# stivalaa/cuda_satabsearch

Measured on AMD Instinct MI355X. Metric: db-structure scorings/sec (query×db pairs/sec) at r=128; 1/2/4/8 MI355X, higher is better.
Workload: dtype i32

## Files before the change

### cuda_satabsearch_amd/build.py

```python
import os
import re
import shutil
import subprocess
import sys

PKG = os.path.dirname(os.path.abspath(__file__))
ROOT = os.path.dirname(PKG)
CSRC = os.path.join(PKG, "csrc")
HOST = os.path.join(CSRC, "host")
INC = os.path.join(ROOT, "include")

HIPCC = os.environ.get("HIPCC") or shutil.which("hipcc") or "/opt/rocm/bin/hipcc"
CC = os.environ.get("CC") or "gcc"


def _run(cmd):
    print("+", " ".join(cmd), flush=True)
    subprocess.run(cmd, check=True)


def _stale(target, sources):
    if not os.path.exists(target):
        return True
    t = os.path.getmtime(target)
    return any(os.path.getmtime(s) > t for s in sources)


DEVICE_SOURCES = ("sat_launch.hip", "sat_capi.hip", "sat_pairs.hip", "sat_db.hip", "sat_topk.hip", "sat_multi.hip",
                  "sat_polish.hip", "sat_qfromdb.hip", "sat_cluster.hip", "sat_eval.hip", "sat_cover.hip", "sat_profile.hip",
                  "sat_reorder.hip", "sat_exact.hip", "sat_reach.hip")
KERNEL_SOURCES = ("sat_sa_kernel.hpp", "sat_sa_body.inc", "sat_launch.hpp", "sat_launch.hip")
HIPFLAGS = ["--offload-arch=gfx950", "-O3", "-ffp-contract=off", "-std=c++17", "-fPIC", "-I", INC, "-I", CSRC]
DEVICE_LIB = (os.path.join(PKG, "libsatabsearch.so"), os.path.join(PKG, "obj", "lib"), [])
SELFCHECK_LIB = (os.path.join(ROOT, "tests", "native", "libsat_selfcheck.so"), os.path.join(PKG, "obj", "selfcheck"),
                 ["-DSAT_DIAG", "-DSAT_DIAG_SELFCHECK"])
JOBS = 16


def kernel_source_hash():
    import hashlib
    h = hashlib.sha256()
    for f in KERNEL_SOURCES:
        with open(os.path.join(CSRC, f), "rb") as fh:
            h.update(fh.read())
    return h.hexdigest()


def include_closure(src):
    seen, todo = [], [src]
    while todo:
        f = todo.pop()
        if f in seen:
            continue
        seen.append(f)
        with open(f) as fh:
            names = re.findall(r'^[ \t]*#[ \t]*include[ \t]+"([^"]+)"', fh.read(), re.M)
        for name in names:
            hits = [p for p in (os.path.normpath(os.path.join(d, name)) for d in (os.path.dirname(f), CSRC, INC)) if os.path.exists(p)]
            todo += hits[:1]
    return seen


def build_host(force=False):
    out = os.path.join(PKG, "libsathost.so")
    srcs = [os.path.join(HOST, f) for f in ("sat_parse.c", "sat_gumbel.c", "sat_shard.c", "sat_cluster.c", "sat_eval.c", "sat_cover.c",
                                            "sat_profile.c", "sat_reorder.c", "sat_exact.c", "sat_reach.c")]
    deps = srcs + [os.path.join(HOST, f) for f in ("sat_parse.h", "sat_gumbel.h", "sat_stats.h", "sat_shard.h", "sat_cluster.h", "sat_eval.h",
                                                "sat_cover.h", "sat_profile.h", "sat_reorder.h", "sat_exact.h", "sat_reach.h")]
    if force or _stale(out, deps):
        _run([CC, "-O2", "-fPIC", "-shared", "-Wall", "-Wextra", "-I", HOST, "-o", out] + srcs + ["-lm", "-lpthread"])
    return out


def _host_objects(force=False):
    host_c = [os.path.join(HOST, "sat_gumbel.c"), os.path.join(HOST, "sat_shard.c"), os.path.join(HOST, "sat_cluster.c"),
              os.path.join(HOST, "sat_eval.c"), os.path.join(HOST, "sat_cover.c"), os.path.join(HOST, "sat_reach.c")]
    host_o = [os.path.join(PKG, "sat_gumbel.o"), os.path.join(PKG, "sat_shard.o"), os.path.join(PKG, "sat_cluster.o"),
              os.path.join(PKG, "sat_eval.o"), os.path.join(PKG, "sat_cover.o"), os.path.join(PKG, "sat_reach.o")]
    for c, o in zip(host_c, host_o):
        if force or _stale(o, [c] + [os.path.join(HOST, h) for h in ("sat_gumbel.h", "sat_stats.h", "sat_shard.h", "sat_cluster.h", "sat_eval.h",
                                                                      "sat_cover.h", "sat_reach.h")]):
            _run([CC, "-O2", "-fPIC", "-ffp-contract=off", "-Wall", "-Wextra", "-I", HOST, "-c", "-o", o, c])
    return host_o


def build_device_libs(libs, force=False):
    host_c = [os.path.join(HOST, f) for f in ("sat_gumbel.c", "sat_shard.c", "sat_cluster.c", "sat_eval.c", "sat_cover.c",
                                              "sat_reach.c", "sat_gumbel.h", "sat_stats.h", "sat_shard.h", "sat_cluster.h",
                                              "sat_eval.h", "sat_cover.h", "sat_reach.h")]
    srcs = [os.path.join(CSRC, f) for f in DEVICE_SOURCES]
    deps = [include_closure(src) for src in srcs]
    todo = [lib for lib in libs if force or _stale(lib[0], host_c + sum(deps, []))]
    if not todo:
        return
    host_o = _host_objects(force)
    compiles = []
    for out, objdir, flags in todo:
        os.makedirs(objdir, exist_ok=True)
    for src, dep in zip(srcs, deps):
        for out, objdir, flags in todo:
            obj = os.path.join(objdir, os.path.splitext(os.path.basename(src))[0] + ".o")
            if force or _stale(obj, dep):
                compiles.append([HIPCC] + HIPFLAGS + flags + ["-c", "-o", obj, src])
    from concurrent.futures import ThreadPoolExecutor
    with ThreadPoolExecutor(JOBS) as ex:
        list(ex.map(_run, compiles))
    for out, objdir, flags in todo:
        objs = [os.path.join(objdir, os.path.splitext(f)[0] + ".o") for f in DEVICE_SOURCES]
        _run([HIPCC, "--offload-arch=gfx950", "-fPIC", "-shared", "-o", out] + ["-Wl," + o for o in objs + host_o] + ["-lm", "-ldl"])


def build_device(force=False):
    build_device_libs([DEVICE_LIB], force)
    return DEVICE_LIB[0]


def build_cli(force=False):
    src = os.path.join(HOST, "sat_main.c")
    if not os.path.exists(src):
        return None
    bindir = os.path.join(PKG, "bin")
    os.makedirs(bindir, exist_ok=True)
    out = os.path.join(bindir, "satabsearch")
    host_search = os.path.join(HOST, "sat_host_search.c")
    deps = [src, host_search, os.path.join(HOST, "sat_host_search.h"), os.path.join(HOST, "sat_cluster.h"),
            os.path.join(HOST, "sat_cover.h"), os.path.join(HOST, "sat_profile.h"), os.path.join(HOST, "sat_reorder.h"),
            os.path.join(PKG, "libsatabsearch.so"), os.path.join(PKG, "libsathost.so")]
    if force or _stale(out, deps):
        _run([CC, "-O3", "-ffp-contract=off", "-Wall", "-Wextra", "-I", INC, "-I", HOST, "-o", out, src, host_search,
              "-L", PKG, "-lsatabsearch", "-lsathost", "-lm", "-Wl,-rpath,$ORIGIN/.."])
    return out


def build_test_native(force=False, twin=True):
    tdir = os.path.join(ROOT, "tests", "native")
    src = os.path.join(tdir, "rocrand_check.hip")
    if not os.path.exists(src):
        return None
    out = os.path.join(tdir, "librocrand_check.so")
    if force or _stale(out, [src, os.path.join(CSRC, "sat_sa_kernel.hpp"), os.path.join(CSRC, "sat_sa_body.inc")]):
        _run([HIPCC, "--offload-arch=gfx950", "-O3", "-std=c++17", "-fPIC", "-shared", "-I", INC, "-I", CSRC, "-o", out, src])
    if twin:
        build_device_libs([SELFCHECK_LIB], force)
    src2, out2 = os.path.join(tdir, "lds_residency.hip"), os.path.join(tdir, "liblds_residency.so")
    if os.path.exists(src2) and (force or _stale(out2, [src2])):
        _run([HIPCC, "--offload-arch=gfx950", "-O2", "-std=c++17", "-fPIC", "-shared", "-o", out2, src2])
    src3, out3 = os.path.join(tdir, "stream_probe.hip"), os.path.join(tdir, "libstream_probe.so")
    if os.path.exists(src3) and (force or _stale(out3, [src3])):
        _run([HIPCC, "--offload-arch=gfx950", "-O2", "-std=c++17", "-fPIC", "-shared", "-o", out3, src3])
    return out


def build_oracle(ref=False):
    odir = os.path.join(ROOT, "oracle")
    _run(["make", "-s", "-C", odir, "all"])
    if ref and os.path.isdir("/root/reference/nvcc_src_current"):
        _run(["make", "-s", "-C", odir, "ref"])


def build_all(force=False, oracle=False, ref=False):
    build_host(force)
    if oracle:
        build_device_libs([DEVICE_LIB, SELFCHECK_LIB], force)
        build_test_native(force, twin=False)
        build_cli(force)
        build_oracle(ref)
    else:
        build_device(force)
        build_cli(force)


if __name__ == "__main__":
    build_all(force="--force" in sys.argv, oracle="--oracle" in sys.argv or "--ref" in sys.argv,
              ref="--ref" in sys.argv)
```

### cuda_satabsearch_amd/csrc/sat_sa_body.inc

```
    using namespace satk;
    constexpr int M1W = (N1P + 31) / 32;
    extern __shared__ __align__(16) unsigned char lds_raw[];

    const int nthreads = a.tpe;
    const int wave_wg = __builtin_amdgcn_readfirstlane((int)(threadIdx.x >> 6));
    const int slot = a.epw > 1 ? wave_wg / (nthreads >> 6) : 0;
    const int wlane = (int)(threadIdx.x & 63u);
    const int lane_id = ((wave_wg - slot * (nthreads >> 6)) << 6) | wlane;
    __builtin_assume(lane_id >= 0 && lane_id < 1024);
    const uint32_t lds_base = (uint32_t)slot * a.lds_stride;
    unsigned char *const lds_slot = lds_raw + lds_base;
    constexpr bool FAST = OPT >= 0;
    const int lpc_shift = FAST ? (OPT >> 2) : a.lpc_shift;
    const bool opt_lorder = FAST ? (OPT & 1) != 0 : a.lorder != 0;
    const bool opt_compact = FAST ? (OPT & 1) != 0 : a.compact != 0;
    const int lpc = 1 << lpc_shift;
    const int tid = lane_id >> lpc_shift;
    const int part = lane_id & (lpc - 1);
    const int T = nthreads >> lpc_shift;
    const int list_pos = (int)blockIdx.x * a.epw + slot;
    SatPairItem pit{};
    if constexpr (PAIRS) pit = px.items[min(list_pos, a.n_list - 1)];
    const int e = PAIRS ? pit.entry : a.entry_list[min(list_pos, a.n_list - 1)];
    const SatQuery Q = PAIRS ? a.queries[pit.desc] : a.queries[blockIdx.y];
// ... 165 lines not shown
        }
        __syncthreads();
    }

    uint8_t *smap_b = reinterpret_cast<uint8_t *>(smap);
    uint8_t *bmap_b = reinterpret_cast<uint8_t *>(bmap);
    auto bmap_byte_addr = [&](int k) -> int { return (__mul24(k >> 2, T) + tid) * 4 + (k & 3); };
    const int T4 = TP << 2, tid4 = tid << 2;
    auto map_byte_addr = [&](int k) -> int { return __mul24(k >> 2, T4) + tid4 + (k & 3); };

    auto score_rows = [&]() -> int {
        int total = 0;
        for (int i = 0; i < n1 - 1; i++) {
            const uint32_t jb = smap_b[map_byte_addr(i)];
            const int j = MAPOFF ? (int)(jb >> 3) : (int)jb;
            const bool jreal = MAPOFF ? (jb & SAT_MAP_UNMATCHED) == 0u : j != NULLJ;
            const DbRow<CELLS> drow = db_row(jreal ? j : 0);
            int rowsum = 0;
            auto row_group = [&](int kw) {
                const int below = i + 1 - 4 * kw;
                const uint32_t force = below <= 0 ? 0u : (0x04040404u >> (8 * (4 - below)));
                const uint32_t qi = (uint32_t)(kw * N1P + i);
                rowsum = quad_terms(load_qdist(qi << 4), load_qcode(qi << 2), drow, smap[kw * TP + tid], force, rowsum);
            };
            if (lpc == 1) {
                for (int kw = (i + 1) >> 2; kw < n1w; kw++) {
                    const int below = i + 1 - 4 * kw;
                    const uint32_t force = below <= 0 ? 0u : (0x04040404u >> (8 * (4 - below)));
                    const uint32_t qi = (uint32_t)(kw * N1P + i);
                    rowsum = quad_terms(load_qdist_uniform(qi), load_qcode_uniform(qi), drow, smap[kw * TP + tid], force, rowsum);
                }
            } else {
                for (int kw = ((i + 1) >> 2) + part; kw < n1w; kw += lpc) row_group(kw);
            }
            total += jreal ? rowsum : 0;
        }
        return total;
    };

    const uint64_t subseq_lo = (uint64_t)a.ordinal[e];
    int best = SAT_K_NO_SCORE;
    uint32_t best_restart = 0xFFFFFFFFu;
    bool any = false;

    const int cmp_recip = (65536 + cmp_lpi - 1) / cmp_lpi;
    const int per_round = (64 * cmp_recip) >> 16;
    const int sub = __mul24(wlane, cmp_recip) >> 16, kw = wlane - __mul24(sub, cmp_lpi);
    const bool lane_ok = sub < per_round;
    const int tail1_recip = (65536 + n1w - 1) / n1w, tail1_rows = (64 * tail1_recip) >> 16;
    const int tail2_lpi = (n1w + 1) >> 1;
    const int tail2_recip = (65536 + tail2_lpi - 1) / tail2_lpi;
    const int tail2_rows = 2 * tail2_lpi <= cmp_words ? (64 * tail2_recip) >> 16 : 0;
    const uint32_t nullword = map_encode<MAPOFF>(NULLJ, NULLJ) * 0x01010101u;
    SAT_PHASE(7);
    SAT_DIAG_PERTURB_INIT;
    size_t mrow = 0;
    uint32_t *mrec = nullptr;
    int r_begin = tid, r_end = a.maxstart;
    if constexpr (PAIRS) {
        r_begin = pit.r0 + tid;
        r_end = pit.r1;
    }
    int rbest = SAT_K_NO_SCORE;
    Bits<M2W> rset = bits_zero<M2W>();
    if constexpr (MATCH) {
        if constexpr (PAIRS) {
            mrow = (size_t)pit.pair;
            mrec = mx.rec_slabs + (size_t)pit.slab * mx.rec_slab_words;
        } else {
            mrow = (size_t)(&a.queries[blockIdx.y] - mx.desc_base) * (size_t)mx.n_entries + (size_t)e;
            mrec = mx.rec_slabs + ((size_t)blockIdx.y * gridDim.x * a.epw + list_pos) * mx.rec_slab_words;
        }
        if (replay) {
            const int cnt = mx.counts[mrow];
            r_begin = tid < cnt ? mx.restarts[mrow * mx.max_matches + tid] : 0;
            r_end = tid < cnt ? r_begin + 1 : 0;
        }
    }
    for (int restart = r_begin; restart < r_end; restart += T) {
        any = true;
        SAT_PHASE(7);
        const uint64_t subseq = subseq_lo | ((uint64_t)(uint32_t)restart << 32);

        Bits<M1W> mapped = bits_zero<M1W>();
        Bits<M2W> occ = bits_zero<M2W>();
        {
            {
                int wa = tid;
                asm volatile("" : "+v"(wa));
                for (int w = 0; w < cmp_words; w++, wa += TP) smap[wa] = nullword;
            }
            int j = 0;
            bool stopped = false;
            for (int i0 = 0; i0 < n1; i0 += 4) {
                if constexpr (N1P > 32)
                    if (__builtin_amdgcn_ballot_w64(!stopped) == 0ull) break;
                uint4 r = philox_block(Q.seed_q, subseq, (uint32_t)(i0 >> 2));
                uint32_t rv[4] = { r.x, r.y, r.z, r.w };
#pragma unroll
                for (int s = 0; s < 4; s++) {
                    const int i = i0 + s;
                    if (i < n1) {
                        if (!stopped && rv[s] < 0x7FFFFFC0u) {
                            Bits<M2W> cand, below = bits_below<M2W>(j);
                            if constexpr (M2W == 1) {
                                cand.w[0] = qmask[i] & ~below.w[0];
                            } else {
                                const int t = qtypes[i];
#pragma unroll
                                for (int w = 0; w < M2W; w++) cand.w[w] = tmask[t * TMS + w] & ~below.w[w];
                            }
                            int jj = bits_lowest<M2W>(cand);
                            if (jj < 0) {
                                stopped = true;
                            } else {
                                smap_b[map_byte_addr(i)] = (uint8_t)(MAPOFF ? jj << 3 : jj);
                                bits_set<M1W>(mapped, i);
                                bits_set<M2W>(occ, jj);
                                j = jj + 1;
                            }
                        }
                    }
                }
            }
        }

        SAT_PHASE(10);
        int score = 0;
        constexpr bool FS_PAIRS = N1P > 16 && !SAT_DIAG_FS_ROWS_ONLY;
        bool walk_pairs = FS_PAIRS;
        if constexpr (FS_PAIRS) {
            constexpr int PAIR_COST = 27;
            const int m = bits_count<M1W>(mapped);
            walk_pairs = __builtin_amdgcn_ballot_w64(__mul24(__mul24(m, m - 1), PAIR_COST) > __mul24(__mul24(n1w, n1), 31)) == 0ull;
        }
        if (walk_pairs) {
            typedef uint32_t u32x2_t __attribute__((ext_vector_type(2)));
            typedef const __attribute__((address_space(1))) u32x2_t *gptr_u2;
            const gptr_c qpairG = (gptr_c)(uintptr_t)Q.qpair;
            constexpr bool POP_IMAGES = M2W == 1;
            static_assert(POP_IMAGES || !MAPOFF, "the walk's map-byte reads take plain indices");
            Bits<M1W> ri = mapped;
            Bits<M2W> rj = occ;
            auto pop = [](auto &b, bool &valid) -> int {
                constexpr int W = sizeof(b.w) / sizeof(b.w[0]);
                valid = bits_any<W>(b);
                const int pos = max(bits_lowest<W>(b), 0);
                bits_drop_lowest<W>(b);
                return pos;
            };
            constexpr bool FS_TEAMS = SAT_FS_TEAMS && M1W == 1 && M2W == 1 && FAST && (OPT == 0 || OPT == 1);
            bool teamed = false;
            if constexpr (FS_TEAMS) teamed = __builtin_amdgcn_ballot_w64(true) == ~0ull;
            if (FS_TEAMS && teamed) {
                const int pl = wlane & 1;
                const uint32_t om = (uint32_t)__shfl_xor((int)mapped.w[0], 1, 64), oo = (uint32_t)__shfl_xor((int)occ.w[0], 1, 64);
                const uint32_t m0 = pl ? om : mapped.w[0], o0 = pl ? oo : occ.w[0];
                const uint32_t m1 = pl ? mapped.w[0] : om, o1 = pl ? occ.w[0] : oo;
                const int c0n = __popc(m0), c1n = __popc(m1);
                const bool big1 = c1n > c0n;
                const uint32_t mb = big1 ? m1 : m0, ob = big1 ? o1 : o0, msm = big1 ? m0 : m1, osm = big1 ? o0 : o1;
                const int rb = max((big1 ? c1n : c0n) - 1, 0), rs = max((big1 ? c0n : c1n) - 1, 0);
                const int dlead = rb - rs, etot = rb + rs;
                uint32_t rm = mb, ro = ob;
                int cur = 0, acc_b = 0, acc_s = 0;
                bool on_small = false;
                for (int e = pl; __builtin_amdgcn_ballot_w64(e < etot) != 0ull; e += 2) {
                    const bool act = e < etot;
                    const int e2 = e - dlead;
                    const bool small = e2 >= 0 && (e2 & 1) != 0;
                    const int len = e2 < 0 ? rb - e : rs - (e2 >> 1);
                    const int a = (small ? rs : rb) - len;
                    if (small && !on_small) { rm = msm; ro = osm; cur = 0; on_small = true; }
#pragma unroll
                    for (int q = 0; q < 2; q++) {
                        const uint32_t go = (act && cur < a) ? 1u : 0u;
                        rm &= rm - go;
                        ro &= ro - go;
                        cur += (int)go;
                    }
                    const int i = act ? __ffs(rm) - 1 : 0, ji = act ? __ffs(ro) - 1 : 0;
                    Bits<1> rk, rl;
                    rk.w[0] = act ? rm & (rm - 1u) : 0u;
                    rl.w[0] = act ? ro & (ro - 1u) : 0u;
                    const DbRow<CELLS> drow = db_row(ji);
                    const uint32_t qrow = (uint32_t)__mul24(i, N1P * 8);
                    int rowsum = 0;
                    while (__builtin_amdgcn_ballot_w64(rk.w[0] != 0u) != 0ull) {
                        int ll[SAT_FS_UNROLL];
                        bool vv[SAT_FS_UNROLL];
                        u32x2_t qcell[SAT_FS_UNROLL];
#pragma unroll
                        for (int u = 0; u < SAT_FS_UNROLL; u++) {
                            bool vl;
                            const int k = pop(rk, vv[u]);
                            ll[u] = pop(rl, vl);
                            qcell[u] = *(gptr_u2)(qpairG + (qrow + ((uint32_t)k << 3)));
                        }
#pragma unroll
                        for (int u = 0; u < SAT_FS_UNROLL; u++) {
                            const uint2 c = db_cell<CELLS>(drow, ll[u]);
                            const int term = pair_term(qcell[u].x, qcell[u].y, c.x, c.y);
                            rowsum += vv[u] ? term : 0;
                        }
                    }
                    acc_s += small ? rowsum : 0;
                    acc_b += small ? 0 : rowsum;
                }
                const int acc0 = big1 ? acc_s : acc_b, acc1 = big1 ? acc_b : acc_s;
                score = (pl ? acc1 : acc0) + __shfl_xor(pl ? acc0 : acc1, 1, 64);
            } else
            while (__builtin_amdgcn_ballot_w64(bits_any<M1W>(ri)) != 0ull) {
                bool ai, aj;
                int i = 0, ji = 0;
                ai = false;
                Bits<M1W> rk = bits_zero<M1W>();
                Bits<M2W> rl = bits_zero<M2W>();
                for (int p = 0; p < lpc; p++) {
                    bool v;
                    const int pos = pop(ri, v);
                    int img = 0;
                    if constexpr (POP_IMAGES) { bool vj; img = pop(rj, vj); }
                    if (p == part) {
                        i = pos;
                        ai = v;
                        ji = img;
                        rk = ri;
                        rl = rj;
                    }
                }
                (void)aj;
                if constexpr (!POP_IMAGES) { ji = smap_b[map_byte_addr(i)]; ji = ai ? ji : 0; }
                const DbRow<CELLS> drow = db_row(ji);
                const uint32_t qrow = (uint32_t)__mul24(i, N1P * 8);
                int rowsum = 0;
                while (__builtin_amdgcn_ballot_w64(bits_any<M1W>(rk)) != 0ull) {
                    int ll[SAT_FS_UNROLL];
                    bool vv[SAT_FS_UNROLL];
                    u32x2_t qcell[SAT_FS_UNROLL];
#pragma unroll
                    for (int u = 0; u < SAT_FS_UNROLL; u++) {
                        const int ku = pop(rk, vv[u]);
                        ll[u] = 0;
                        if constexpr (POP_IMAGES) { bool vl; ll[u] = pop(rl, vl); }
                        if constexpr (!POP_IMAGES) ll[u] = smap_b[map_byte_addr(ku)];
                        qcell[u] = *(gptr_u2)(qpairG + (qrow + ((uint32_t)ku << 3)));
                    }
#pragma unroll
                    for (int u = 0; u < SAT_FS_UNROLL; u++) {
                        const uint2 c = db_cell<CELLS>(drow, ll[u]);
                        const int term = pair_term(qcell[u].x, qcell[u].y, c.x, c.y);
                        rowsum += vv[u] ? term : 0;
                    }
                }
                score += rowsum;
            }
        } else {
            score = score_rows();
        }
        if (lpc >= 2) score += __shfl_xor(score, 1, 64);
        if (lpc == 4) score += __shfl_xor(score, 2, 64);
        const int best_before = best;
        if (score > best) {
            best = score;
            if (lsoln && beats_leader(score, restart))
                for (int w = 0; w < n1w; w++) bmap[w * T + tid] = smap[w * TP + tid];
        }
        if constexpr (MATCH) {
            rbest = score;
            rset = occ;
            if (replay && part == 0)
                for (int w = 0; w < n1w; w++) bmap[w * T + tid] = smap[w * TP + tid];
        }

        SAT_PHASE(6);
        uint4 blk = uint4{ 0u, 0u, 0u, 0u };
        for (int iter = 0; iter < SAT_K_MAXITER; iter++) {
            const int rowoff = prowC[2 * iter], rowmax = prowC[2 * iter + 1];
            constexpr bool ROW_IN_LANES = N1P >= 32 && M2W == 1 && (OPT < 0 || (OPT & 1) != 0);
            float rowv = 0.0f;
            if constexpr (ROW_IN_LANES)
                rowv = *(gptr_f32)((gptr_c)ptabG + (((uint32_t)rowoff + (uint32_t)min(wlane, rowmax + 2)) << 2));
            if ((iter & 1) == 0) {
                blk = philox_block(Q.seed_q, subseq, (uint32_t)(SAT_K_STEP_BLOCK0 + (iter >> 1)));
            } else {
                blk.x = blk.z;
                blk.y = blk.w;
            }
            const uint32_t word_a = blk.x, word_b = blk.y;
            SAT_DIAG_PERTURB_STEP;

            const int ssei = scaled_index16(word_a >> 16, n1, n1 - 1);

            int oldj;
            Bits<M2W> cand;
            int rank_base = 0;
            if (M2W == 1 && opt_lorder) {
                int p;
                bool none;
                highest_mapped_upto(mapped, ssei, p, none);
                const int A = MAPOFF ? smap_b[map_byte_addr(p)] >> 3 : smap_b[map_byte_addr(p)];
                SAT_DIAG_DUP_MAPBYTE(&smap_b[map_byte_addr(p)]);
                oldj = (p == ssei && !(MAPOFF && none)) ? A : NULLJ;
                const uint32_t above = 0xFFFFFFFEu << (A & 31);
                const uint32_t y = occ.w[0] & above;
                const uint32_t gap = (y - 1u) & ~y & above;
                const bool empty = none || (y == 0u && ssei != n1 - 1);
// ... 390 lines not shown
```

### cuda_satabsearch_amd/csrc/sat_sa_kernel.hpp

```cpp
#pragma once

#include <hip/hip_runtime.h>
#include <type_traits>
#include <stdint.h>

#ifdef SAT_DIAG
#include "diag/sat_diag.hpp"
#endif
#ifndef SAT_DIAG_ARGS
#define SAT_DIAG_ARGS
#endif
#ifndef SAT_PHASE_INIT
#define SAT_PHASE_INIT
#define SAT_PHASE(k)
#define SAT_PHASE_FLUSH
#endif
#ifndef SAT_DIAG_FS_ROWS_ONLY
#define SAT_DIAG_FS_ROWS_ONLY 0
#endif
#ifndef SAT_DIAG_DUP_CELLS
#define SAT_DIAG_DUP_CELLS(row, o0, o1, o2, o3)
#endif
#ifndef SAT_DIAG_DUP_MAPWORD
#define SAT_DIAG_DUP_MAPWORD(p)
#endif
#ifndef SAT_DIAG_DUP_ATOMIC
#define SAT_DIAG_DUP_ATOMIC(p)
#endif
#ifndef SAT_DIAG_DUP_MAPBYTE
#define SAT_DIAG_DUP_MAPBYTE(p)
#endif
#ifndef SAT_DIAG_PERTURB_INIT
#define SAT_DIAG_PERTURB_INIT
#define SAT_DIAG_PERTURB_STEP
#define SAT_DIAG_PERTURB_END
#endif
#ifndef SAT_DIAG_SELFCHECK_STEP
#define SAT_DIAG_SELFCHECK_STEP
#endif

#define SAT_CELLS_FULL8 0
#define SAT_CELLS_FULL5 1
#define SAT_CELLS_TRI5  2
#ifndef SAT_FAST_WAVES
#define SAT_FAST_WAVES 6
#endif
#ifndef SAT_FS_TEAMS
#define SAT_FS_TEAMS 1
#endif
#ifndef SAT_PICK_TABLE
#define SAT_PICK_TABLE 1
#endif
#define SAT_K_MAXITER 100
#define SAT_K_MAXDIM 111
#define SAT_FS_UNROLL 2
#define SAT_K_STEP_BLOCK0 32
#define SAT_K_EPS 1.1e-7
#define SAT_K_NO_SCORE (-99999)
#define SAT_K_QSENT 1.0e30f
#define SAT_K_DSENT (-1.0e30f)

struct SatQuery {
    const float4   *qdist;
    const uint32_t *qcode;
    const uint8_t  *qtypes;
    const uint2    *qpair;
    int32_t         n1;
    uint32_t        pad_;
    uint64_t        seed_q;
    int32_t        *scores;
    int8_t         *ssemaps;
};

struct SatKernelArgs {
    const int32_t  *orders;
    const int64_t  *cell_off;
    const uint8_t  *tab_tri;
    const float    *dist_tri;
    const uint32_t *ordinal;
    const int32_t  *entry_list;
    int32_t         n_list;
    int32_t         epw, tpe;
    uint32_t        lds_stride;
    const SatQuery *queries;
    int32_t         lorder, lsoln, maxstart;
    int32_t         lpc_shift;
    int32_t         compact;
    uint32_t       *bmap_slabs;
    uint32_t        bmap_slab_words;
    const float    *ptab;
    const int32_t  *prow;
    SAT_DIAG_ARGS
};

struct SatMatchArgs {
    const SatQuery *desc_base;
    int32_t         n_entries;
    int32_t         max_matches;
    int32_t         replay;
    int32_t         map_pitch;
    uint32_t       *rec_slabs;
    uint32_t        rec_slab_words;
    uint32_t        pad_;
    int32_t        *counts;
    int32_t        *scores;
    int32_t        *restarts;
    int8_t         *maps;
};

struct SatPairItem {
    int32_t pair;
    int32_t desc;
    int32_t entry;
    int32_t r0, r1;
    int32_t slab;
    int32_t pad_[2];
};
struct SatPairArgs {
    const SatPairItem   *items;
    unsigned long long  *keys;
    int8_t              *maps;
};

namespace satk {

template <int W> struct Bits { uint32_t w[W]; };

template <int W> __device__ __forceinline__ Bits<W> bits_zero()
{
    Bits<W> b;
#pragma unroll
    for (int i = 0; i < W; i++) b.w[i] = 0u;
    return b;
}
template <int W> __device__ __forceinline__ Bits<W> bits_below(int pos)
{
    Bits<W> b;
    if constexpr (W == 1) {
        const int s = 32 - min(max(pos, 0), 32);
        const int h = s >> 1;
        b.w[0] = (0xFFFFFFFFu >> h) >> (s - h);
        return b;
    }
    const int wi = pos >> 5;
    const uint32_t part = (1u << (pos & 31)) - 1u;
#pragma unroll
    for (int i = 0; i < W; i++) b.w[i] = i < wi ? 0xFFFFFFFFu : (i == wi ? part : 0u);
    return b;
}
template <int W> __device__ __forceinline__ void bits_set(Bits<W> &b, int pos)
{
#pragma unroll
    for (int i = 0; i < W; i++) b.w[i] |= ((pos >> 5) == i) ? (1u << (pos & 31)) : 0u;
}
template <int W> __device__ __forceinline__ void bits_clear(Bits<W> &b, int pos)
{
#pragma unroll
    for (int i = 0; i < W; i++) b.w[i] &= ~(((pos >> 5) == i) ? (1u << (pos & 31)) : 0u);
}
template <int W> __device__ __forceinline__ int bits_count(const Bits<W> &b)
{
    int c = 0;
#pragma unroll
    for (int i = 0; i < W; i++) c += __popc(b.w[i]);
    return c;
}
template <int W> __device__ __forceinline__ bool bits_any(const Bits<W> &b)
{
    uint32_t o = 0u;
#pragma unroll
    for (int i = 0; i < W; i++) o |= b.w[i];
    return o != 0u;
}
template <int W> __device__ __forceinline__ void bits_drop_lowest(Bits<W> &b)
{
    bool done = false;
#pragma unroll
    for (int i = 0; i < W; i++) {
        const bool here = !done && b.w[i] != 0u;
        b.w[i] = here ? b.w[i] & (b.w[i] - 1u) : b.w[i];
        done = done || here;
    }
}
template <int W> __device__ __forceinline__ int bits_lowest(const Bits<W> &b)
{
    int r = -1;
#pragma unroll
    for (int i = W - 1; i >= 0; i--) r = b.w[i] ? 32 * i + (__ffs(b.w[i]) - 1) : r;
    return r;
}
template <int W> __device__ __forceinline__ int bits_highest(const Bits<W> &b)
{
    int r = -1;
#pragma unroll
    for (int i = 0; i < W; i++) r = b.w[i] ? 32 * i + (31 - __clz(b.w[i])) : r;
    return r;
}
__device__ __forceinline__ int word_select(uint32_t v, int r)
{
    uint32_t a = v - ((v >> 1) & 0x55555555u);
    uint32_t b = (a & 0x33333333u) + ((a >> 2) & 0x33333333u);
// ... 149 lines not shown
        const uint64_t p0 = (uint64_t)0xD2511F53u * c0, p1 = (uint64_t)0xCD9E8D57u * c2;
        uint32_t n0, n2;
        if (r < 3) {
            n0 = (uint32_t)(p1 >> 32) ^ c1 ^ k0;
            n2 = (uint32_t)(p0 >> 32) ^ c3 ^ k1;
        } else {
            n0 = __builtin_amdgcn_bitop3_b32((uint32_t)(p1 >> 32), c1, k0, 0x96);
            n2 = __builtin_amdgcn_bitop3_b32((uint32_t)(p0 >> 32), c3, k1, 0x96);
        }
        c1 = (uint32_t)p1;
        c3 = (uint32_t)p0;
        c0 = n0;
        c2 = n2;
        k0 += 0x9E3779B9u;
        k1 += 0xBB67AE85u;
    }
    return uint4{ c0, c1, c2, c3 };
}
__device__ __forceinline__ float draw32(uint32_t v)
{
    return (float)v + 1.0f;
}
__device__ __forceinline__ float to_uniform(uint32_t v)
{
    return draw32(v) * 2.3283064365386963e-10f;
}
__device__ __forceinline__ int scaled_index16(uint32_t v16, int n, int nm1)
{
    return (int)(__umul24(v16, (uint32_t)n) + (uint32_t)nm1) >> 16;
}

__host__ __device__ inline void compaction_shape(int n1w, int &lpi, int &wpl)
{
    lpi = (n1w + 3) >> 2;
    wpl = lpi > 0 ? (n1w + lpi - 1) / lpi : 1;
    if (lpi < 1) lpi = 1;
}
__host__ __device__ inline int map_words(int n1w)
{
    int lpi, wpl;
    compaction_shape(n1w, lpi, wpl);
    return lpi * wpl;
}

struct LdsLayout {
    uint32_t code;
    uint32_t qdist;
    uint32_t qcode;
    uint32_t smap;
    uint32_t tmask;
    uint32_t qtypes;
    uint32_t qmask;
    uint32_t qbase;
    uint32_t pos;
    uint32_t leader;
    uint32_t red;
    uint32_t red_stride;
    uint32_t items;
    uint32_t total;
};
__host__ __device__ inline LdsLayout lds_layout(int m2w, int cells, int n2, int words, int n1p, int chains, int threads,
                                                 bool q_in_lds, bool compact)
{
    LdsLayout L;
    const bool split = cells != SAT_CELLS_FULL8;
    uint32_t dcells = (uint32_t)n2 * (uint32_t)(n2 + 1);
    uint32_t off;
    if (split) {
        if (cells == SAT_CELLS_TRI5) dcells = tri_cells(n2);
        dcells = (dcells + 3u) & ~3u;
        L.code = dcells * 4u;
        off = L.code + ((dcells + 15u) & ~15u);
    } else {
        dcells = (dcells + 1u) & ~1u;
        L.code = 0u;
        off = dcells * 8u;
    }
    L.qdist = off;
    if (q_in_lds) off += (uint32_t)words * (uint32_t)n1p * 16u;
    L.qcode = off;
    if (q_in_lds) off += (uint32_t)words * (uint32_t)n1p * 4u;
    L.smap = off;
    off += (((uint32_t)words * (uint32_t)(chains + 1) + 1u) & ~1u) * 4u;
    L.tmask = off;
    off += 4u * (uint32_t)m2w * 4u;
    L.qtypes = off;
    off += ((uint32_t)n1p + 15u) & ~15u;
    L.qmask = off;
    if (m2w == 1) off += (uint32_t)n1p * 4u;
    L.qbase = off;
    if (m2w == 1) off += (uint32_t)n1p;
    L.pos = off;
    if (m2w == 1) off += SAT_POS_BYTES;
    off = (off + 7u) & ~7u;
    L.leader = off;
    off += 8u;
    L.red = off;
    L.red_stride = compact ? 256u : 8u;
    if (!compact) off += 16u * 8u;
    L.items = off;
    if (compact) off += (uint32_t)((threads + 63) / 64) * 64u * 4u;
    L.total = off;
    return L;
}

__host__ __device__ inline size_t lds_bytes(int n1, int n1p, int n2, int chains, int threads, bool lsoln, bool q_in_lds,
                                             bool compact)
{
    (void)lsoln;
    return lds_layout(set_words(n2), cell_layout(n2), n2, map_words((n1 + 3) >> 2), n1p, chains, threads, q_in_lds, compact).total;
}

}


template <int N1P, int M2W, bool QLDS, int OPT, int WPL, int CELLS>
__global__ void __launch_bounds__(1024) __attribute__((amdgpu_waves_per_eu((OPT < 0 || OPT >= 4) ? 4 : SAT_FAST_WAVES)))
sat_sa_kernel(const SatKernelArgs a)
{
    constexpr bool MATCH = false, PAIRS = false;
    const SatMatchArgs mx{};
    const SatPairArgs px{};
#include "sat_sa_body.inc"
}

template <int N1P, int M2W, bool QLDS, int CELLS>
__global__ void __launch_bounds__(1024) __attribute__((amdgpu_waves_per_eu(4)))
sat_sa_match_kernel(const SatKernelArgs a, const SatMatchArgs mx)
{
    constexpr bool MATCH = true, PAIRS = false;
    constexpr int OPT = -1, WPL = 0;
    const SatPairArgs px{};
#include "sat_sa_body.inc"
}

template <int N1P, int M2W, bool QLDS, int OPT, int CELLS>
__global__ void __launch_bounds__(1024) __attribute__((amdgpu_waves_per_eu((OPT < 0 || OPT >= 4) ? 4 : SAT_FAST_WAVES)))
sat_sa_pair_kernel(const SatKernelArgs a, const SatPairArgs px)
{
    constexpr bool MATCH = false, PAIRS = true;
    constexpr int WPL = 0;
    const SatMatchArgs mx{};
#include "sat_sa_body.inc"
}

template <int N1P, int M2W, bool QLDS, int CELLS>
__global__ void __launch_bounds__(1024) __attribute__((amdgpu_waves_per_eu(4)))
sat_sa_pair_match_kernel(const SatKernelArgs a, const SatPairArgs px, const SatMatchArgs mx)
{
    constexpr bool MATCH = true, PAIRS = true;
    constexpr int OPT = -1, WPL = 0;
#include "sat_sa_body.inc"
}
```

Before: 12.35 million.

## Flatten full-score pair work across the whole wave with prefix-sum load balancing

Adds a new full-score path for OPT==1 that compacts the lanes with nonzero work, prefix-sums their pair counts with DPP, and splits the total pair work into equal chunks per lane. Each lane seeks to its starting pair, walks its chunk with a cursor, and accumulates terms into per-owner LDS slots using wavefront-scope atomics. This replaces the two-lane team walk, which was limited by the largest lane in the wave. In exchange it adds permutes, a binary search, LDS atomics and wave barriers. The old team path stays available through a build flag.

```diff
diff --git a/cuda_satabsearch_amd/build.py b/cuda_satabsearch_amd/build.py
--- a/cuda_satabsearch_amd/build.py
+++ b/cuda_satabsearch_amd/build.py
@@ -34,6 +34,8 @@
 DEVICE_LIB = (os.path.join(PKG, "libsatabsearch.so"), os.path.join(PKG, "obj", "lib"), [])
 SELFCHECK_LIB = (os.path.join(ROOT, "tests", "native", "libsat_selfcheck.so"), os.path.join(PKG, "obj", "selfcheck"),
                  ["-DSAT_DIAG", "-DSAT_DIAG_SELFCHECK"])
+TEAMWALK_LIB = (os.path.join(ROOT, "tests", "native", "libsat_teamwalk.so"), os.path.join(PKG, "obj", "teamwalk"),
+                ["-DSAT_FS_FLAT=0"])
 JOBS = 16
 
 
@@ -161,7 +163,7 @@
 def build_all(force=False, oracle=False, ref=False):
     build_host(force)
     if oracle:
-        build_device_libs([DEVICE_LIB, SELFCHECK_LIB], force)
+        build_device_libs([DEVICE_LIB, SELFCHECK_LIB, TEAMWALK_LIB], force)
         build_test_native(force, twin=False)
         build_cli(force)
         build_oracle(ref)
diff --git a/cuda_satabsearch_amd/csrc/sat_sa_body.inc b/cuda_satabsearch_amd/csrc/sat_sa_body.inc
--- a/cuda_satabsearch_amd/csrc/sat_sa_body.inc
+++ b/cuda_satabsearch_amd/csrc/sat_sa_body.inc
@@ -341,7 +341,71 @@
             constexpr bool FS_TEAMS = SAT_FS_TEAMS && M1W == 1 && M2W == 1 && FAST && (OPT == 0 || OPT == 1);
             bool teamed = false;
             if constexpr (FS_TEAMS) teamed = __builtin_amdgcn_ballot_w64(true) == ~0ull;
-            if (FS_TEAMS && teamed) {
+            constexpr bool FS_FLAT = SAT_FS_FLAT && FS_TEAMS && OPT == 1;
+            if (FS_FLAT && teamed) {
+                const uint32_t mp = mapped.w[0], oc = occ.w[0];
+                const bool owns = (mp & (mp - 1u)) != 0u;
+                const unsigned long long nzb = __builtin_amdgcn_ballot_w64(owns);
+                const int NZ = __popcll(nzb);
+                const int rank = __builtin_amdgcn_mbcnt_hi((uint32_t)(nzb >> 32), __builtin_amdgcn_mbcnt_lo((uint32_t)nzb, 0));
+                const int dest = (owns ? rank : NZ + wlane - rank) << 2;
+                uint32_t cm = (uint32_t)__builtin_amdgcn_ds_permute(dest, (int)mp), co = (uint32_t)__builtin_amdgcn_ds_permute(dest, (int)oc);
+                cm = wlane < NZ ? cm : SAT_FS_DUMMY_SET;
+                co = wlane < NZ ? co : SAT_FS_DUMMY_SET;
+                const int p = wlane < NZ ? fs_pairs(cm) : 0;
+                int incl = p;
+                incl += __builtin_amdgcn_update_dpp(0, incl, 0x111, 0xF, 0xF, false);
+                incl += __builtin_amdgcn_update_dpp(0, incl, 0x112, 0xF, 0xF, false);
+                incl += __builtin_amdgcn_update_dpp(0, incl, 0x114, 0xF, 0xF, false);
+                incl += __builtin_amdgcn_update_dpp(0, incl, 0x118, 0xF, 0xF, false);
+                incl += __builtin_amdgcn_update_dpp(0, incl, 0x142, 0xA, 0xF, false);
+                incl += __builtin_amdgcn_update_dpp(0, incl, 0x143, 0xC, 0xF, false);
+                const int P = __builtin_amdgcn_readlane(incl, 63);
+                const int q = fs_chunk(P);
+                const int first = __mul24(wlane, q), mine = fs_chunk_pairs(P, q, wlane);
+                int r = 0;
+#pragma unroll
+                for (int d = 32; d > 0; d >>= 1) {
+                    const int s = __builtin_amdgcn_ds_bpermute((r + d) << 2, incl - p);
+                    r = s <= first ? r + d : r;
+                }
+                const int s0 = __builtin_amdgcn_ds_bpermute(r << 2, incl - p);
+                FsCursor cur = fs_seek((uint32_t)__builtin_amdgcn_ds_bpermute(r << 2, (int)cm),
+                                       (uint32_t)__builtin_amdgcn_ds_bpermute(r << 2, (int)co), mine > 0 ? first - s0 : 0);
+                items[wlane] = 0u;
+                __builtin_amdgcn_fence(__ATOMIC_RELEASE, "wavefront");
+                __builtin_amdgcn_wave_barrier();
+                __builtin_amdgcn_fence(__ATOMIC_ACQUIRE, "wavefront");
+                for (int it = 0; it < q; it += SAT_FS_UNROLL) {
+                    int ll[SAT_FS_UNROLL], rr[SAT_FS_UNROLL];
+                    bool vv[SAT_FS_UNROLL];
+                    DbRow<CELLS> drow[SAT_FS_UNROLL];
+                    u32x2_t qcell[SAT_FS_UNROLL];
+#pragma unroll
+                    for (int u = 0; u < SAT_FS_UNROLL; u++) {
+                        vv[u] = it + u < mine;
+                        const int i = __builtin_ctz(cur.rm), k = __builtin_ctz(cur.rk);
+                        drow[u] = db_row(__builtin_ctz(cur.ro));
+                        ll[u] = __builtin_ctz(cur.rl);
+                        rr[u] = r;
+                        qcell[u] = *(gptr_u2)(qpairG + ((uint32_t)__mul24(i, N1P * 8) + ((uint32_t)k << 3)));
+                        const uint32_t nm = (uint32_t)__builtin_amdgcn_ds_bpermute((r + 1) << 2, (int)cm);
+                        const uint32_t no = (uint32_t)__builtin_amdgcn_ds_bpermute((r + 1) << 2, (int)co);
+                        r += fs_advance(cur, vv[u] ? 1u : 0u, nm, no) ? 1 : 0;
+                    }
+#pragma unroll
+                    for (int u = 0; u < SAT_FS_UNROLL; u++) {
+                        const uint2 c = db_cell<CELLS>(drow[u], ll[u]);
+                        int term = pair_term(qcell[u].x, qcell[u].y, c.x, c.y);
+                        asm volatile("" : "+v"(term));
+                        if (vv[u]) __hip_atomic_fetch_add((lds_i32_t *)(items + rr[u]), term, __ATOMIC_RELAXED, __HIP_MEMORY_SCOPE_WAVEFRONT);
+                    }
+                }
+                __builtin_amdgcn_fence(__ATOMIC_RELEASE, "wavefront");
+                __builtin_amdgcn_wave_barrier();
+                __builtin_amdgcn_fence(__ATOMIC_ACQUIRE, "wavefront");
+                score = owns ? (int)items[rank] : 0;
+            } else if (FS_TEAMS && teamed) {
                 const int pl = wlane & 1;
                 const uint32_t om = (uint32_t)__shfl_xor((int)mapped.w[0], 1, 64), oo = (uint32_t)__shfl_xor((int)occ.w[0], 1, 64);
                 const uint32_t m0 = pl ? om : mapped.w[0], o0 = pl ? oo : occ.w[0];
diff --git a/cuda_satabsearch_amd/csrc/sat_sa_kernel.hpp b/cuda_satabsearch_amd/csrc/sat_sa_kernel.hpp
--- a/cuda_satabsearch_amd/csrc/sat_sa_kernel.hpp
+++ b/cuda_satabsearch_amd/csrc/sat_sa_kernel.hpp
@@ -1,8 +1,77 @@
 #pragma once
 
+#ifndef SAT_FS_CHUNKS_ONLY
 #include <hip/hip_runtime.h>
 #include <type_traits>
+#endif
 #include <stdint.h>
+
+#if defined(__HIPCC__)
+#define SAT_FS_HD __host__ __device__ __forceinline__
+#else
+#define SAT_FS_HD inline
+#endif
+
+namespace satk {
+
+#define SAT_FS_DUMMY_SET 3u
+
+SAT_FS_HD int fs_pairs(uint32_t mapped)
+{
+    const int m = __builtin_popcount(mapped);
+    return (m * (m - 1)) >> 1;
+}
+SAT_FS_HD int fs_chunk(int P) { return (P + 63) >> 6; }
+SAT_FS_HD int fs_chunk_pairs(int P, int q, int t)
+{
+    const int left = P - t * q;
+    return left < 0 ? 0 : (left < q ? left : q);
+}
+
+struct FsCursor { uint32_t rm, ro, rk, rl; };
+
+SAT_FS_HD FsCursor fs_seek(uint32_t mapped, uint32_t occ, int off)
+{
+    FsCursor c;
+    c.rm = mapped;
+    c.ro = occ;
+    int len = __builtin_popcount(mapped) - 1;
+    while (off >= len && len > 1) {
+        off -= len;
+        len--;
+        c.rm &= c.rm - 1u;
+        c.ro &= c.ro - 1u;
+    }
+    c.rk = c.rm & (c.rm - 1u);
+    c.rl = c.ro & (c.ro - 1u);
+    while (off > 0 && (c.rk & (c.rk - 1u)) != 0u) {
+        off--;
+        c.rk &= c.rk - 1u;
+        c.rl &= c.rl - 1u;
+    }
+    return c;
+}
+
+SAT_FS_HD bool fs_advance(FsCursor &c, uint32_t go, uint32_t nm, uint32_t no)
+{
+    c.rk &= c.rk - go;
+    c.rl &= c.rl - go;
+    const bool row_end = c.rk == 0u;
+    const uint32_t e = row_end ? 1u : 0u;
+    uint32_t rm = c.rm & (c.rm - e), ro = c.ro & (c.ro - e);
+    const bool chain_end = row_end && (rm & (rm - 1u)) == 0u;
+    rm = chain_end ? nm : rm;
+    ro = chain_end ? no : ro;
+    c.rm = rm;
+    c.ro = ro;
+    c.rk = row_end ? rm & (rm - 1u) : c.rk;
+    c.rl = row_end ? ro & (ro - 1u) : c.rl;
+    return chain_end;
+}
+
+}
+
+#ifndef SAT_FS_CHUNKS_ONLY
 
 #ifdef SAT_DIAG
 #include "diag/sat_diag.hpp"
@@ -47,6 +116,9 @@
 #endif
 #ifndef SAT_FS_TEAMS
 #define SAT_FS_TEAMS 1
+#endif
+#ifndef SAT_FS_FLAT
+#define SAT_FS_FLAT 1
 #endif
 #ifndef SAT_PICK_TABLE
 #define SAT_PICK_TABLE 1
@@ -502,3 +574,5 @@
     constexpr int OPT = -1, WPL = 0;
 #include "sat_sa_body.inc"
 }
+
+#endif
```

After: 13.09 million, median of 6. 1.06x the previous value.
